# nianticlabs/simplerecon

Measured on AMD Instinct MI355X. Metric: depth frames/sec (640x480, 7 src views, 64 planes), higher is better.
Workload: dtype f32

## Files before the change

include/simplerecon_hip.h:

```cpp
#ifndef SIMPLERECON_HIP_H_
#define SIMPLERECON_HIP_H_

#include <stddef.h>
#include <stdint.h>

#ifdef __cplusplus
extern "C" {
#endif

#define SR_OK 0
#define SR_ERR_INVALID_ARGUMENT 1
#define SR_ERR_UNSUPPORTED 2
#define SR_ERR_WORKSPACE_TOO_SMALL 3
#define SR_ERR_HIP_BASE 1000

enum {
  SR_OPT_MLP_SPLIT = 0, SR_OPT_WINO_SPLIT, SR_OPT_WINO_XCD, SR_OPT_WINO_NT, SR_OPT_WINO_KSPLIT, SR_OPT_CONV_WINO,
  SR_OPT_CONV_TILE, SR_OPT_CONV_KSPLIT, SR_OPT_PW_NT, SR_OPT_PW_KS, SR_OPT_PT_CFG, SR_OPT_PT_KS, SR_OPT_DOT_LDS,
  SR_OPT_DOT_LDS_G, SR_OPT_DOT_LDS_CULL, SR_OPT_DOT_LDS_CAP, SR_OPT_UPSAMPLE_QUAD, SR_OPT_POOL_STREAM,
  SR_OPT_COUNT
};
int sr_option_count(void);
const char* sr_option_name(int id);
int sr_option_id(const char* name);
int sr_option_get(int id, int* value);
int sr_option_set(int id, int value, int* previous );
int sr_option_default(int id, int* value);

int sr_abi_version(void);

const char* sr_target_arch(void);


size_t sr_volume_workspace_bytes(int B, int K, int C, int h, int w);

int sr_volume_prepare(const float* src, const float* K_src, const float* T_src_cur,
                      const float* T_cur_src, int B, int K, int C, int h, int w, void* workspace,
                      size_t workspace_bytes, void* stream);

int sr_dot_volume_sweep(const float* cur, const float* invK_cur, const float* planes, int64_t ps_b,
                        int64_t ps_d, int64_t ps_y, int64_t ps_x, int B, int K, int C, int h, int w,
                        int D, float* out_cv, int64_t cv_sb, int64_t cv_sd, int64_t cv_sp,
                        float* out_lowest, uint8_t* out_mask, void* workspace,
                        size_t workspace_bytes, void* stream);

int sr_conv3x3_wino_io_nhwc_fwd(const void* in, int64_t in_batch_stride, int in_pix_stride, const float* packed_u,
                                const float* bias, const void* residual, int64_t res_batch_stride, int res_pix_stride,
                                void* out, int64_t out_batch_stride, int out_pix_stride, int B, int H, int W, int Cin,
                                int Cout, float leaky_slope, int io_dtype, void* stream);
int sr_pw_conv_io_nhwc_fwd(const void* in, int64_t in_batch_stride, int in_pix_stride, const float* packed_w,
                           const float* bias, const void* residual, int64_t res_batch_stride, int res_pix_stride, void* out,
                           int64_t out_batch_stride, int out_pix_stride, int B, int HW, int Cin, int Cout, float act_code,
                           int io_dtype, void* stream);

size_t sr_pw_conv_tiled_workspace_bytes(int M, int Cin, int Cout);
int sr_pw_conv_tiled_plan(int M, int Cin, int Cout, int can_split, int* cfg, int* ks);
int sr_pw_conv_tiled_nhwc_fwd(const float* in, int in_pix_stride, const float* packed_w, const float* bias,
                              const float* gate, const float* residual, int res_pix_stride, float* out,
                              int out_pix_stride, int M, int HW, int Cin, int Cout, float act_code, void* workspace,
                              size_t workspace_bytes, void* stream);
int sr_pw_conv_supported(int Cin, int Cout);
int sr_pw_conv_plan(int B, int HW, int Cin, int Cout, int* nt, int* ks);
int sr_pw_conv_nhwc_fwd(const float* in, int64_t in_batch_stride, int in_pix_stride, const float* packed_w,
                        const float* bias, const float* gate, const float* residual, int64_t res_batch_stride,
                        int res_pix_stride, float* out, int64_t out_batch_stride, int out_pix_stride, int B, int HW,
                        int Cin, int Cout, float act_code, void* stream);

int sr_backproject_fwd(const float* depth, const float* invK, float* out_points, int B, int h, int w, void* stream);
int sr_project3d_fwd(const float* points, const float* K, const float* T, float* out, int B, int N, float eps,
                     void* stream);
int sr_backproject_bwd(const float* grad_points, const float* invK, float* grad_depth, int B, int h, int w, void* stream);
int sr_project3d_bwd(const float* grad_out, const float* points, const float* K, const float* T, float* grad_points, int B,
// ... 416 lines not shown
```

simplerecon_amd/csrc/sr_options.hip:

```cpp
#include <atomic>
#include <mutex>
#include <stdlib.h>
#include <string.h>

#include "sr_common.h"

namespace {

struct OptDef { const char* name; int dflt; int kind; };
const OptDef kDefs[SR_OPT_COUNT] = {
    {"SR_MLP_SPLIT", 0, 1},       {"SR_WINO_SPLIT", 0, 1},     {"SR_WINO_XCD", 1, 0},        {"SR_WINO_NT", 0, 0},
    {"SR_WINO_KSPLIT", 0, 0},     {"SR_CONV_WINO", 1, 0},      {"SR_CONV_TILE", 0, 0},       {"SR_CONV_KSPLIT", 1, 0},
    {"SR_PW_NT", 0, 0},           {"SR_PW_KS", 0, 0},          {"SR_PT_CFG", -1, 0},         {"SR_PT_KS", 0, 0},
    {"SR_DOT_LDS", 1, 0},         {"SR_DOT_LDS_G", 0, 0},      {"SR_DOT_LDS_CULL", 1, 0},    {"SR_DOT_LDS_CAP", 634, 0},
    {"SR_UPSAMPLE_QUAD", 1, 0},   {"SR_POOL_STREAM", 1, 0},
};
std::atomic<int> g_val[SR_OPT_COUNT];
std::once_flag g_once;

int parse(const OptDef& d, const char* e) {
  if (d.kind == 1) {
    if (!e || !*e || !strcmp(e, "0") || !strcmp(e, "off") || !strcmp(e, "fp32")) return 0;
    if (!strcmp(e, "bf16")) return 1;
    if (!strcmp(e, "f16") || !strcmp(e, "fp16")) return 2;
    return -1;
  }
  return (e && *e) ? atoi(e) : d.dflt;
}

void init() {
  for (int i = 0; i < SR_OPT_COUNT; ++i) {
    const char* e = getenv(kDefs[i].name);
    g_val[i].store(e ? parse(kDefs[i], e) : kDefs[i].dflt, std::memory_order_relaxed);
  }
}

}

int sr_opt(int id) {
  std::call_once(g_once, init);
  return g_val[id].load(std::memory_order_relaxed);
}

extern "C" int sr_option_count(void) { return SR_OPT_COUNT; }

extern "C" const char* sr_option_name(int id) { return (id >= 0 && id < SR_OPT_COUNT) ? kDefs[id].name : nullptr; }

extern "C" int sr_option_id(const char* name) {
  if (!name) return -1;
  for (int i = 0; i < SR_OPT_COUNT; ++i)
    if (!strcmp(kDefs[i].name, name)) return i;
  return -1;
}

extern "C" int sr_option_get(int id, int* value) {
  if (id < 0 || id >= SR_OPT_COUNT || !value) return SR_ERR_INVALID_ARGUMENT;
  *value = sr_opt(id);
  return SR_OK;
}

extern "C" int sr_option_set(int id, int value, int* previous) {
  if (id < 0 || id >= SR_OPT_COUNT) return SR_ERR_INVALID_ARGUMENT;
  std::call_once(g_once, init);
  const int old = g_val[id].exchange(value, std::memory_order_relaxed);
  if (previous) *previous = old;
  return SR_OK;
}

// ... 19 lines not shown
```

simplerecon_amd/csrc/sr_pw.hip:

```cpp
#include <stdlib.h>

#include "sr_common.h"

namespace {

typedef float pw_f16 __attribute__((ext_vector_type(16)));
typedef float pw_f4 __attribute__((ext_vector_type(4)));
typedef unsigned int pw_u4 __attribute__((ext_vector_type(4)));
#define PW_RSRC_FLAGS 0x00020000
#define PW_OOB 0x7fffffffu

__device__ __forceinline__ pw_f4 pw_load(__amdgpu_buffer_rsrc_t r, unsigned voff, unsigned soff) {
  return __builtin_bit_cast(pw_f4, __builtin_amdgcn_raw_buffer_load_b128(r, (int)voff, (int)soff, 0));
}
typedef unsigned int pw_u2 __attribute__((ext_vector_type(2)));
template <int IO>
__device__ __forceinline__ float pw_widen(unsigned short h) {
  if (IO == 1) return (float)__builtin_bit_cast(_Float16, h);
  return __builtin_bit_cast(float, (unsigned)h << 16);
}
template <int IO>
__device__ __forceinline__ unsigned short pw_narrow(float f) {
  if (IO == 1) return __builtin_bit_cast(unsigned short, (_Float16)f);
  return __builtin_bit_cast(unsigned short, (__bf16)f);
}
template <int IO>
__device__ __forceinline__ pw_f4 pw_load_a(__amdgpu_buffer_rsrc_t r, unsigned voff, unsigned soff) {
  if (IO == 0) return __builtin_bit_cast(pw_f4, __builtin_amdgcn_raw_buffer_load_b128(r, (int)voff, (int)soff, 0));
  const pw_u2 v = __builtin_bit_cast(pw_u2, __builtin_amdgcn_raw_buffer_load_b64(r, (int)voff, (int)soff, 0));
  return pw_f4{pw_widen<IO>((unsigned short)(v.x & 0xffffu)), pw_widen<IO>((unsigned short)(v.x >> 16)),
               pw_widen<IO>((unsigned short)(v.y & 0xffffu)), pw_widen<IO>((unsigned short)(v.y >> 16))};
}
template <int IO>
__device__ __forceinline__ float pw_load_elem(__amdgpu_buffer_rsrc_t r, unsigned voff, unsigned soff) {
  if (IO == 0) return __builtin_bit_cast(float, __builtin_amdgcn_raw_buffer_load_b32(r, (int)voff, (int)soff, 0));
  return pw_widen<IO>(__builtin_amdgcn_raw_buffer_load_b16(r, (int)voff, (int)soff, 0));
}
template <int IO>
__device__ __forceinline__ void pw_store_elem(float v, __amdgpu_buffer_rsrc_t r, unsigned voff, unsigned soff) {
  if (IO == 0) __builtin_amdgcn_raw_buffer_store_b32(__builtin_bit_cast(unsigned, v), r, (int)voff, (int)soff, 0);
  else __builtin_amdgcn_raw_buffer_store_b16(pw_narrow<IO>(v), r, (int)voff, (int)soff, 0);
}
#define PW_ES(io) ((io) == 0 ? 4u : 2u)

__device__ __forceinline__ __amdgpu_buffer_rsrc_t pw_rsrc(const void* base, int64_t bytes) {
  return __builtin_amdgcn_make_buffer_rsrc(const_cast<void*>(base), 0, (int)bytes, PW_RSRC_FLAGS);
}

struct SrPwParams {
  const float* in; int64_t in_sb; int in_sp;
  const float* wp;
  const float* bias;
  const float* gate;
  const float* res; int64_t res_sb; int res_sp;
  float* out; int64_t out_sb; int out_sp;
  int B, HW, Cin, Cout, Co_pad, G, G8;
  int m_tiles, n_blocks, total_mt;
  float slope;
};

#ifndef SR_PW_U
#define SR_PW_U 4
#define SR_PW_PD 3
#endif
constexpr int PW_U = SR_PW_U;
constexpr int PW_PD = SR_PW_PD;

template <int NT, int KS, bool GATE, int IO = 0>
__global__ __launch_bounds__(256, 2) void sr_pw_kernel(SrPwParams p) {
  constexpr unsigned ES = PW_ES(IO);
  extern __shared__ __attribute__((aligned(16))) float red[];
  const int tid = threadIdx.x;
  const int lane = tid & 63, wave = __builtin_amdgcn_readfirstlane(tid >> 6);
  const int i = lane & 31, kk = lane >> 5;
  constexpr int MT_PER_WG = 4 / KS;
  const int ml = wave / KS, kp = wave % KS;
  const int item = blockIdx.x;
  const int nb = item % p.n_blocks;
  const int mt_g = (item / p.n_blocks) * MT_PER_WG + ml;
  const bool live = mt_g < p.total_mt;
  const int img = live ? mt_g / p.m_tiles : 0;
  const int row0 = live ? (mt_g - img * p.m_tiles) * 32 : 0;
  const int n0 = nb * (32 * NT);

  const int per = ((p.G8 + KS - 1) / KS + PW_U - 1) / PW_U * PW_U;
  const int g0 = kp * per;
  const int g1 = min(p.G8, g0 + per);
  const int steps = live && g1 > g0 ? (g1 - g0 + PW_U - 1) / PW_U * PW_U : 0;

  const __amdgpu_buffer_rsrc_t rs_in = pw_rsrc(reinterpret_cast<const char*>(p.in) + (int64_t)img * p.in_sb * ES,
                                               ((int64_t)(p.HW - 1) * p.in_sp + p.Cin) * ES);
  const __amdgpu_buffer_rsrc_t rs_w = pw_rsrc(p.wp, (int64_t)p.G * 2 * p.Co_pad * 16);
  const __amdgpu_buffer_rsrc_t rs_g = pw_rsrc(GATE ? p.gate + (int64_t)img * p.Cin : p.wp, GATE ? (int64_t)p.Cin * 4 : 0);
  const int row = row0 + i;
  const unsigned a_voff = (row < p.HW) ? ((unsigned)row * (unsigned)p.in_sp + 4u * kk) * ES : PW_OOB;
  const bool k_tail = (p.Cin & 7) != 0;
  const unsigned w_voff = (unsigned)(kk * p.Co_pad + n0 + i) * 16u;
  const unsigned g_voff = 16u * kk;
  const int g_last_w = p.G - 1;

  pw_f16 acc[NT];
#pragma unroll
  for (int n = 0; n < NT; ++n)
#pragma unroll
    for (int r = 0; r < 16; ++r) acc[n][r] = 0.0f;

  pw_f4 a_f[PW_U], b_f[PW_U][NT], s_f[PW_U];
  auto issue = [&](int g, int slot) {
    const bool in_range = g < g1;
    unsigned av = in_range ? a_voff : PW_OOB;
    if (k_tail && 8 * g + 4 * kk + 4 > p.Cin) av = PW_OOB;
    a_f[slot] = pw_load_a<IO>(rs_in, av, (unsigned)g * 8u * ES);
    if (GATE) s_f[slot] = pw_load(rs_g, g_voff + (unsigned)g * 32u, 0u);
    const unsigned gw = (unsigned)min(g, g_last_w);
#pragma unroll
    for (int n = 0; n < NT; ++n) b_f[slot][n] = pw_load(rs_w, w_voff + 512u * n, gw * 2u * (unsigned)p.Co_pad * 16u);
  };
  if (steps > 0) {
#pragma unroll
    for (int s = 0; s < PW_PD; ++s) issue(g0 + s, s);
  }
  for (int gb = 0; gb < steps; gb += PW_U) {
#pragma unroll
    for (int u = 0; u < PW_U; ++u) {
      issue(g0 + gb + u + PW_PD, (u + PW_PD) % PW_U);
      pw_f4 a = a_f[u];
      if (GATE) a = a * s_f[u];
#pragma unroll
      for (int e = 0; e < 4; ++e)
#pragma unroll
        for (int n = 0; n < NT; ++n) acc[n] = __builtin_amdgcn_mfma_f32_32x32x2f32(a[e], b_f[u][n][e], acc[n], 0, 0, 0);
    }
  }

  if (KS > 1) {
    if (kp > 0 && live) {
#pragma unroll
      for (int n = 0; n < NT; ++n)
// ... 170 lines not shown
```

simplerecon_amd/csrc/sr_pw_tiled.hip:

```cpp
#include <stdlib.h>

#include "sr_common.h"

namespace {

typedef float pt_f16 __attribute__((ext_vector_type(16)));
typedef float pt_f4 __attribute__((ext_vector_type(4)));

constexpr int PT_KS = 32;
constexpr int PT_AROW = PT_KS + 4;

struct SrPtParams {
  const float* in; int in_sp;
  const float* wp;
  const float* bias; const float* gate;
  const float* res; int res_sp;
  float* out; int out_sp;
  int64_t part_stride;
  int M, HW, Cin, Cout, Co_pad, G;
  int slabs, slabs_per_part, ksplit, tiles_n;
  float slope;
};

template <int WM, int WN, int NTW, bool GATE>
__global__ __launch_bounds__(256, 2) void sr_pw_tiled_kernel(SrPtParams p) {
  constexpr int BM = 32 * WM, BN = 32 * WN * NTW;
  constexpr int A_FLOATS = BM * PT_AROW, B_FLOATS = (PT_KS / 8) * 2 * BN * 4;
  constexpr int A_PER_THREAD = BM * (PT_KS / 4) / 256;
  constexpr int B_PER_THREAD = (PT_KS / 8) * 2 * BN / 256;
  static_assert(WM * WN == 4 && A_PER_THREAD >= 1 && B_PER_THREAD >= 1, "4 waves; whole float4s per thread");
  extern __shared__ __attribute__((aligned(16))) float lds[];
  const int tid = threadIdx.x, lane = tid & 63, wave = __builtin_amdgcn_readfirstlane(tid >> 6);
  const int i = lane & 31, kk = lane >> 5;
  const int wm = wave / WN, wn = wave % WN;
  const int tile_n = blockIdx.x % p.tiles_n, tile_m = blockIdx.x / p.tiles_n;
  const int kpart = blockIdx.y;
  const int m0 = tile_m * BM, n0 = tile_n * BN;
  const int s_begin = kpart * p.slabs_per_part, s_end = min(p.slabs, s_begin + p.slabs_per_part);

  int a_row[A_PER_THREAD];
  const float* a_ptr[A_PER_THREAD];
  const float* g_ptr[A_PER_THREAD];
  const int a_q = tid & 7;
#pragma unroll
  for (int u = 0; u < A_PER_THREAD; ++u) {
    a_row[u] = (tid >> 3) + 32 * u;
    const int m = m0 + a_row[u];
    const bool ok = m < p.M;
    a_ptr[u] = ok ? p.in + (int64_t)m * p.in_sp + 4 * a_q : nullptr;
    g_ptr[u] = (GATE && ok) ? p.gate + (int64_t)(m / p.HW) * p.Cin + 4 * a_q : nullptr;
  }
  auto stage_load = [&](int s, pt_f4 (&ra)[A_PER_THREAD], pt_f4 (&rb)[B_PER_THREAD]) {
    const int k0 = s * PT_KS;
#pragma unroll
    for (int u = 0; u < A_PER_THREAD; ++u) {
      pt_f4 v = {0.f, 0.f, 0.f, 0.f};
      if (a_ptr[u] && k0 + 4 * a_q < p.Cin) {
        v = *reinterpret_cast<const pt_f4*>(a_ptr[u] + k0);
        if (GATE) v = v * *reinterpret_cast<const pt_f4*>(g_ptr[u] + k0);
      }
      ra[u] = v;
    }
#pragma unroll
    for (int u = 0; u < B_PER_THREAD; ++u) {
      const int e = tid + 256 * u;
      const int gh = e / BN, col = e - gh * BN;
      const int g = s * (PT_KS / 8) + (gh >> 1);
      pt_f4 v = {0.f, 0.f, 0.f, 0.f};
      if (g < p.G && n0 + col < p.Co_pad)
        v = *reinterpret_cast<const pt_f4*>(p.wp + ((int64_t)(g * 2 + (gh & 1)) * p.Co_pad + n0 + col) * 4);
      rb[u] = v;
    }
  };
  auto stage_store = [&](int buf, const pt_f4 (&ra)[A_PER_THREAD], const pt_f4 (&rb)[B_PER_THREAD]) {
    float* A = lds + buf * (A_FLOATS + B_FLOATS);
    float* Bt = A + A_FLOATS;
#pragma unroll
    for (int u = 0; u < A_PER_THREAD; ++u) *reinterpret_cast<pt_f4*>(&A[a_row[u] * PT_AROW + 4 * a_q]) = ra[u];
#pragma unroll
    for (int u = 0; u < B_PER_THREAD; ++u) *reinterpret_cast<pt_f4*>(&Bt[(tid + 256 * u) * 4]) = rb[u];
  };

  pt_f16 acc[NTW];
#pragma unroll
  for (int n = 0; n < NTW; ++n)
#pragma unroll
    for (int r = 0; r < 16; ++r) acc[n][r] = 0.0f;

  pt_f4 ra[A_PER_THREAD], rb[B_PER_THREAD];
  if (s_begin < s_end) {
    stage_load(s_begin, ra, rb);
    stage_store(0, ra, rb);
  }
  __syncthreads();
  for (int s = s_begin; s < s_end; ++s) {
    const int buf = (s - s_begin) & 1;
    const bool more = s + 1 < s_end;
    if (more) stage_load(s + 1, ra, rb);
    const float* A = lds + buf * (A_FLOATS + B_FLOATS);
    const float* Bt = A + A_FLOATS;
    const float* a_base = A + (32 * wm + i) * PT_AROW + 4 * kk;
    const float* b_base = Bt + (kk * BN + 32 * wn * NTW + i) * 4;
#pragma unroll
    for (int gl = 0; gl < PT_KS / 8; ++gl) {
      const pt_f4 a = *reinterpret_cast<const pt_f4*>(a_base + 8 * gl);
      pt_f4 b[NTW];
#pragma unroll
      for (int n = 0; n < NTW; ++n) b[n] = *reinterpret_cast<const pt_f4*>(b_base + (gl * 2 * BN + 32 * n) * 4);
#pragma unroll
      for (int e = 0; e < 4; ++e)
#pragma unroll
        for (int n = 0; n < NTW; ++n) acc[n] = __builtin_amdgcn_mfma_f32_32x32x2f32(a[e], b[n][e], acc[n], 0, 0, 0);
    }
    if (more) stage_store(buf ^ 1, ra, rb);
    __syncthreads();
  }

  const bool partial = p.ksplit > 1;
  const float slope = sr_uniform(partial ? -1.0f : p.slope);
  float* outp = p.out + (partial ? (int64_t)kpart * p.part_stride : (int64_t)0);
  const int rbase = m0 + 32 * wm + 4 * kk;
#pragma unroll
  for (int n = 0; n < NTW; ++n) {
    const int col = n0 + 32 * (wn * NTW + n) + i;
    const bool okc = col < p.Cout;
    const float bv = (!partial && p.bias && okc) ? p.bias[col] : 0.0f;
    float v[16];
#pragma unroll
    for (int r = 0; r < 16; ++r) v[r] = acc[n][r] + bv;
    if (!partial && p.res) {
      float rv[16];
#pragma unroll
      for (int r = 0; r < 16; ++r) {
        const int m = rbase + (r & 3) + 8 * (r >> 2);
        rv[r] = (okc && m < p.M) ? p.res[(int64_t)m * p.res_sp + col] : 0.0f;
      }
#pragma unroll
      for (int r = 0; r < 16; ++r) v[r] += rv[r];
    }
    sr_activate_group(v, slope);
#pragma unroll
    for (int r = 0; r < 16; ++r) {
      const int m = rbase + (r & 3) + 8 * (r >> 2);
      if (okc && m < p.M) outp[(int64_t)m * p.out_sp + col] = v[r];
    }
  }
}

int pt_num_cus() { return sr_device_cus(); }

struct PtPlan { int cfg, ks; };
constexpr int PT_BM[4] = {64, 128, 128, 64}, PT_BN[4] = {128, 160, 64, 64};

PtPlan pt_plan(int M, int Cin, int Cout, bool can_split) {
  const int f_cfg = sr_opt(SR_OPT_PT_CFG), f_ks = sr_opt(SR_OPT_PT_KS);
  const int slabs = (Cin + PT_KS - 1) / PT_KS;
  const long want = (long)pt_num_cus() * 3 / 2;
  PtPlan best = {0, 1};
  double best_cost = -1.0;
  for (int cfg = 0; cfg < 4; ++cfg) {
    if (f_cfg >= 0 && cfg != f_cfg) continue;
    const long tm = (M + PT_BM[cfg] - 1) / PT_BM[cfg], tn = (Cout + PT_BN[cfg] - 1) / PT_BN[cfg];
    const double pad = (double)(tm * PT_BM[cfg]) * (double)(tn * PT_BN[cfg]) / ((double)M * Cout);
    for (int ks = 1; ks <= 8; ks *= 2) {
      if (f_ks > 0 && ks != f_ks) continue;
      if (ks > 1 && (!can_split || slabs / ks < 4)) continue;
      const long wgs = tm * tn * ks;
      const double fill = wgs >= want ? 1.0 : (double)want / (double)wgs;
      const double reuse = 1.0 + 24.0 / (PT_BM[cfg] * PT_BN[cfg] / (double)(PT_BM[cfg] + PT_BN[cfg]));
      const double cost = pad * fill * reuse * (1.0 + (ks > 1 ? 0.10 + 2.0 * ks / slabs : 0.0));
      if (best_cost < 0 || cost < best_cost) { best = {cfg, ks}; best_cost = cost; }
    }
  }
  return best;
}

template <int WM, int WN, int NTW>
int pt_launch(const SrPtParams& p, int tiles_m, hipStream_t stream) {
  constexpr int BM = 32 * WM, BN = 32 * WN * NTW;
  const size_t lds = (size_t)2 * (BM * PT_AROW + (PT_KS / 8) * 2 * BN * 4) * sizeof(float);
  const dim3 grid((unsigned)(tiles_m * p.tiles_n), (unsigned)p.ksplit);
  if (p.gate) {
    hipError_t e = hipFuncSetAttribute((const void*)sr_pw_tiled_kernel<WM, WN, NTW, true>,
                                       hipFuncAttributeMaxDynamicSharedMemorySize, (int)lds);
    if (e != hipSuccess) return sr_hip_rc(e);
    hipLaunchKernelGGL((sr_pw_tiled_kernel<WM, WN, NTW, true>), grid, dim3(256), lds, stream, p);
  } else {
    hipError_t e = hipFuncSetAttribute((const void*)sr_pw_tiled_kernel<WM, WN, NTW, false>,
                                       hipFuncAttributeMaxDynamicSharedMemorySize, (int)lds);
    if (e != hipSuccess) return sr_hip_rc(e);
    hipLaunchKernelGGL((sr_pw_tiled_kernel<WM, WN, NTW, false>), grid, dim3(256), lds, stream, p);
  }
  return sr_hip_rc(hipGetLastError());
}

}

extern "C" size_t sr_pw_conv_tiled_workspace_bytes(int M, int Cin, int Cout) {
  if (M <= 0 || Cin <= 0 || Cout <= 0 || Cout % 4 != 0) return 0;
  const PtPlan pl = pt_plan(M, Cin, Cout, true);
  return pl.ks > 1 ? (size_t)pl.ks * M * Cout * sizeof(float) : 0;
}

extern "C" int sr_pw_conv_tiled_plan(int M, int Cin, int Cout, int can_split, int* cfg, int* ks) {
  if (M <= 0 || Cin <= 0 || Cout <= 0) return SR_ERR_INVALID_ARGUMENT;
  const PtPlan pl = pt_plan(M, Cin, Cout, can_split != 0 && Cout % 4 == 0);
  if (cfg) *cfg = pl.cfg;
  if (ks) *ks = pl.ks;
  return SR_OK;
}

extern "C" int sr_pw_conv_tiled_nhwc_fwd(const float* in, int in_pix_stride, const float* packed_w, const float* bias,
                                         const float* gate, const float* residual, int res_pix_stride, float* out,
                                         int out_pix_stride, int M, int HW, int Cin, int Cout, float act_code,
                                         void* workspace, size_t workspace_bytes, void* stream_) {
  if (M < 0 || HW <= 0 || Cin <= 0 || Cout <= 0) return SR_ERR_INVALID_ARGUMENT;
  if (M == 0) return SR_OK;
  if (!in || !packed_w || !out) return SR_ERR_INVALID_ARGUMENT;
  if (Cin % 4 != 0 || in_pix_stride % 4 != 0 || (((uintptr_t)in) & 15) != 0 || (gate && (((uintptr_t)gate) & 15) != 0))
    return SR_ERR_UNSUPPORTED;
  const bool can_split = workspace && (((uintptr_t)workspace) & 15) == 0 && Cout % 4 == 0 &&
                         (!residual || ((((uintptr_t)residual) & 15) == 0 && res_pix_stride % 4 == 0)) &&
                         (((uintptr_t)out) & 15) == 0 && out_pix_stride % 4 == 0 && (!bias || (((uintptr_t)bias) & 15) == 0);
  PtPlan pl = pt_plan(M, Cin, Cout, can_split);
  if (pl.ks > 1 && workspace_bytes < (size_t)pl.ks * M * Cout * sizeof(float)) pl = pt_plan(M, Cin, Cout, false);
  SrPtParams p;
  p.in = in; p.in_sp = in_pix_stride; p.wp = packed_w; p.bias = bias; p.gate = gate;
  p.res = residual; p.res_sp = res_pix_stride;
  p.M = M; p.HW = HW; p.Cin = Cin; p.Cout = Cout;
  p.Co_pad = ((Cout + 31) / 32) * 32;
  p.G = ((Cin + 63) / 64) * 8;
  p.slabs = (Cin + PT_KS - 1) / PT_KS;
  p.ksplit = pl.ks;
  p.slabs_per_part = (p.slabs + pl.ks - 1) / pl.ks;
  p.slope = act_code;
  p.part_stride = (int64_t)M * Cout;
  if (pl.ks > 1) { p.out = (float*)workspace; p.out_sp = Cout; }
  else { p.out = out; p.out_sp = out_pix_stride; }
  const int tiles_m = (M + PT_BM[pl.cfg] - 1) / PT_BM[pl.cfg];
  p.tiles_n = (Cout + PT_BN[pl.cfg] - 1) / PT_BN[pl.cfg];
  hipStream_t stream = (hipStream_t)stream_;
  int rc;
  switch (pl.cfg) {
    case 0: rc = pt_launch<2, 2, 2>(p, tiles_m, stream); break;
    case 1: rc = pt_launch<4, 1, 5>(p, tiles_m, stream); break;
    case 2: rc = pt_launch<4, 1, 2>(p, tiles_m, stream); break;
    default: rc = pt_launch<2, 2, 1>(p, tiles_m, stream); break;
  }
  if (rc == SR_OK && pl.ks > 1)
    rc = sr_launch_splitk_reduce((const float*)workspace, pl.ks, p.part_stride, bias, residual, (int64_t)0, res_pix_stride,
                                 out, (int64_t)0, out_pix_stride, 1, M, Cout, act_code, stream);
  return rc;
}
```

simplerecon_amd/ops.py:

```python
import ctypes as C
import contextlib
import os
import weakref

import torch
from torch import nn

from . import _lib

PROFILE = None

_PACKED = weakref.WeakKeyDictionary()
_NO_ENTRIES = {}


def _cached(mod, tag, key, build, *args):
    e = _PACKED.get(mod, _NO_ENTRIES).get(tag)
    if e is not None and e[0] == key:
        if e[2] is not None:
            _await_pack(e)
        return e[1]
    payload = build(*args)
    fence = None
    if _lib.cuda_available() and not _lib.capturing():
# ... 91 lines not shown
        return (w._version, w.data_ptr(), b._version, b.data_ptr())
    ts = [w] if b is None else [w, b]
    bufs, bp = bn._buffers, bn._parameters
    ts += [bufs["running_mean"], bufs["running_var"]]
    if bn.affine:
        ts += [bp["weight"], bp["bias"]]
    return tuple((t._version, t.data_ptr()) if t is not None else None for t in ts)


def bn_affine(bn):
    if bn.running_mean is None or bn.running_var is None:
        raise _lib.HipLibraryError("BatchNorm without running statistics cannot run in inference mode")
    scale = torch.rsqrt(bn.running_var.detach() + bn.eps)
    if bn.affine:
        scale = scale * bn.weight.detach()
    shift = -bn.running_mean.detach() * scale
    if bn.affine:
        shift = shift + bn.bias.detach()
    return scale.contiguous(), shift.contiguous()


def _effective_weight(conv, bn):
    w = conv.weight.detach()
    b = conv.bias.detach() if conv.bias is not None else None
    if bn is not None:
        scale, shift = bn_affine(bn)
        w = w * scale.view(-1, 1, 1, 1)
        b = shift if b is None else b * scale + shift
    return w.contiguous(), b


def _check_conv(conv):
    k = conv.kernel_size[0]
    if conv.kernel_size[0] != conv.kernel_size[1] or k not in (1, 3) or conv.groups != 1 \
            or conv.dilation != (1, 1) or tuple(conv.padding) != (k // 2,) * 2 \
            or conv.padding_mode not in ("zeros", "replicate"):
        raise _lib.HipLibraryError(f"unsupported Conv2d configuration for the HIP path: {conv}")


def _pack_folded(kind, conv, bn):
    _lib.require_device_f32("conv weight", conv.weight)
    _check_conv(conv)
    w, bias = _effective_weight(conv, bn)
    return _pack(kind, w), bias


def packed_weight(conv: nn.Conv2d, bn=None):
    return _cached(conv, "direct", _state_key(conv, bn), _pack_folded, "conv", conv, bn)


USE_PW_1X1 = True
PW_TILED = os.environ.get("SR_PW_TILED", "auto")
PW_TILED_MIN_ROWS = 100000


def _pack_linear(lin):
    return _pack("conv", lin.weight.detach().reshape(lin.out_features, lin.in_features, 1, 1).contiguous())


def linear(x, lin: nn.Linear, leaky=None):
    _lib.require_device_f32("linear input", x)
    _lib.refuse_autograd(x, lin.weight)
    cin, cout = lin.in_features, lin.out_features
    if x.shape[-1] != cin:
        raise ValueError(f"linear expects {cin} input features, got {x.shape[-1]}")
    x2 = x.reshape(-1, cin).contiguous()
    m = x2.shape[0]
    out = torch.empty((m, cout), dtype=torch.float32, device=x.device)
    if m == 0:
        return out.view(*x.shape[:-1], cout)
    wp = _cached(lin, "linear", _state_key(lin, None), _pack_linear, lin)
    bias = lin.bias.detach() if lin.bias is not None else None
    _lib.call("sr_conv2d_nhwc_fwd", x.device, x2, m * cin, cin, wp, bias, None, 0, 0, out, m * cout, cout, 1, 1, m, cin, cout,
              1, 1, -1.0 if leaky is None else float(leaky))
    return out.view(*x.shape[:-1], cout)


def wino_split_mode():
    return _lib.split_mode_name("SR_WINO_SPLIT")


def packed_wino_weight(conv: nn.Conv2d, bn=None):
    key = (_state_key(conv, bn), wino_split_mode())
    return _cached(conv, "wino", key, _pack_folded, "wino", conv, bn)


WINO4_MODE = int(os.environ.get("SR_CONV_WINO4", "1"))
WINO4_VARIANT = int(os.environ.get("SR_WINO4_VARIANT", "0"))


def packed_wino4_weight(conv: nn.Conv2d, bn=None):
    return _cached(conv, "wino4", _state_key(conv, bn), _pack_folded, "wino4", conv, bn)


_SHAPE_QUERIES = {}


def _drop_shape_queries(*_):
    _SHAPE_QUERIES.clear()


_lib.OPTION_LISTENERS.append(_drop_shape_queries)


def _shape_query(lib, name, *shape, dev=None):
    key = (name, shape, dev)
# ... 72 lines not shown
            if _conv_wino(lib, x, *packed_wino_weight(conv, bn), residual, out, strides, shape, slope) == 0:
                return out
        finally:
            _lib.SPLIT_GUARD.release()
        wp, bias = packed_weight(conv, bn)
        isb, isp, osb, osp, rsb, rsp = strides
        _lib.call("sr_conv2d_nhwc_fwd", x.device, x, isb, isp, wp, bias, residual, rsb, rsp, out, osb, osp, b, h, w, ci, co,
                  k, s, slope)
        return out
    _conv_direct(lib, x, *packed_weight(conv, bn), residual, out, strides, shape, slope, pads if padded else None, replicate)
    return out


def _aligned16(t, sb, sp):
    return t is None or (t.data_ptr() % 16 == 0 and sp % 4 == 0 and sb % 4 == 0)


def _timed(device, record, fn, *args):
    prof = PROFILE
    with _lib.on_device(device):
        if prof is None:
            return fn(*args)
        ev0, ev1 = torch.cuda.Event(enable_timing=True), torch.cuda.Event(enable_timing=True)
        ev0.record()
        rc = fn(*args)
        ev1.record()
        if rc == 0:
            name, flops, shape, executed = record()
            prof.append((name, flops, ev0, ev1, shape, executed))
    return rc


def _launch(x, shape, entry, fallback, describe, fn, *args):
    if PROFILE is None:
        with _lib.on_device(x.device):
            rc = fn(*args)
    else:
        def record():
            b, ci, h, w, co, k, s, ho, wo, _ = shape
            name, executed = describe()
            return name, 2.0 * b * ho * wo * co * ci * k * k, shape, executed
        rc = _timed(x.device, record, fn, *args)
    if rc != 0 and (rc != _lib.ERR_UNSUPPORTED or not fallback):
        _lib.check(rc, entry)
    return rc


def _conv_pointwise(lib, x, wp, bias, residual, out, gate, strides, shape, slope):
    isb, isp, osb, osp, rsb, rsp = strides
    b, ci, h, w, co = shape[:5]
    m = b * h * w
    dense = b == 1 or (isb == h * w * isp and osb == h * w * osp and (residual is None or rsb == h * w * rsp))
    gflag = "true" if gate is not None else "false"
    if dense and (PW_TILED == "1" or (PW_TILED == "auto" and m >= PW_TILED_MIN_ROWS)):
        nbytes = _shape_query(lib, "sr_pw_conv_tiled_workspace_bytes", m, ci, co, dev=x.device.index)
        ws = _workspace(x.device, "pw_splitk", nbytes) if nbytes else None

        def describe():
            a_, b_ = C.c_int(0), C.c_int(0)
            can_split = ws is not None and ws.data_ptr() % 16 == 0 and co % 4 == 0 and _aligned16(out, 0, osp) and \
                _aligned16(residual, 0, rsp) and (bias is None or bias.data_ptr() % 16 == 0)
            lib.sr_pw_conv_tiled_plan(m, ci, co, int(can_split), C.byref(a_), C.byref(b_))
            if b_.value > 1 and nbytes < b_.value * m * co * 4:
                lib.sr_pw_conv_tiled_plan(m, ci, co, 0, C.byref(a_), C.byref(b_))
            tile_m, tile_n = ((64, 128), (128, 160), (128, 64), (64, 64))[a_.value]
            executed = 2.0 * (-(-m // tile_m) * tile_m) * (-(-co // tile_n) * tile_n) * (-(-ci // 32) * 32)
            return f"sr_pw_tiled_kernel<{tile_m}x{tile_n}, ks {b_.value}, {gflag}>", executed
        return _launch(x, shape, "sr_pw_conv_tiled_nhwc_fwd", gate is None, describe, lib.sr_pw_conv_tiled_nhwc_fwd,
                       _lib.ptr(x), isp, _lib.ptr(wp), _lib.ptr(bias), _lib.ptr(gate), _lib.ptr(residual), rsp, _lib.ptr(out),
                       osp, m, h * w, ci, co, slope, _lib.ptr(ws), nbytes, _lib.stream_ptr(x.device))

    def describe():
        a_, b_ = C.c_int(0), C.c_int(0)
        lib.sr_pw_conv_plan(b, h * w, ci, co, C.byref(a_), C.byref(b_))
        mt = b * ((h * w + 31) // 32)
        executed = 2.0 * mt * 32 * ((co + 32 * a_.value - 1) // (32 * a_.value) * 32 * a_.value) * ((ci + 7) // 8 * 8)
        return f"sr_pw_kernel<{a_.value}, {b_.value}, {gflag}>", executed
    return _launch(x, shape, "sr_pw_conv_nhwc_fwd", gate is None, describe, lib.sr_pw_conv_nhwc_fwd, _lib.ptr(x), isb, isp,
                   _lib.ptr(wp), _lib.ptr(bias), _lib.ptr(gate), _lib.ptr(residual), rsb, rsp, _lib.ptr(out), osb, osp, b,
                   h * w, ci, co, slope, _lib.stream_ptr(x.device))


def _conv_wino4(lib, x, wp, bias, residual, out, strides, shape, slope, variant):
    isb, isp, osb, osp, rsb, rsp = strides
    b, ci, h, w, co = shape[:5]
    if not (_aligned16(x, isb, isp) and _aligned16(out, osb, osp) and _aligned16(residual, rsb, rsp)
            and (bias is None or bias.data_ptr() % 16 == 0)):
        return _lib.ERR_UNSUPPORTED

    def describe():
        regions = ((h + 15) // 16) * ((w + 15) // 16)
        executed = 2.0 * b * regions * 16 * 36 * ((ci + 15) // 16 * 16) * ((co + 63) // 64 * 64)
        return "sr_wino4ws_kernel" if variant == 3 else "sr_wino4_kernel", executed
    return _launch(x, shape, "sr_conv3x3_wino4_nhwc_fwd", True, describe, lib.sr_conv3x3_wino4_variant_nhwc_fwd, _lib.ptr(x),
                   isb, isp, _lib.ptr(wp), _lib.ptr(bias), _lib.ptr(residual), rsb, rsp, _lib.ptr(out), osb, osp, b, h, w, ci,
                   co, slope, variant, _lib.stream_ptr(x.device))


def _conv_wino(lib, x, wp, bias, residual, out, strides, shape, slope, workspace=True, fallback=True):
    isb, isp, osb, osp, rsb, rsp = strides
    b, ci, h, w, co = shape[:5]
    split = wino_split_mode()
    nbytes = _shape_query(lib, "sr_wino_splitk_workspace_bytes", b, h, w, ci, co, dev=x.device.index) if workspace else 0
    ws = _workspace(x.device, "wino_splitk", nbytes) if nbytes else None

    def describe():
        vin = bool(_aligned16(x, isb, isp) and ci % 4 == 0)
# ... 401 lines not shown
```

Measured before the change: 313.6.

## Rework tiled pointwise conv pipeline, planner cost model, and gated routing

Adds a configurable register-set prefetch depth to the tiled pointwise kernel. Loads become unconditional with clamped addresses and masking moves to the LDS store. The tile/split-k planner gets a new analytic cost model that tries every ks from 1 to 8, and hipFuncSetAttribute is cached per device. Gated 1x1 convs with large Cin and mid-size M are now routed to the tiled kernel, and the simple pw kernel's K-partition alignment is decoupled from its unroll factor. Default depth stays 1, so the main default-path changes are the restructured load/store masking, the new planner and the new routing.

```diff
diff --git a/include/simplerecon_hip.h b/include/simplerecon_hip.h
--- a/include/simplerecon_hip.h
+++ b/include/simplerecon_hip.h
@@ -18,6 +18,7 @@
   SR_OPT_MLP_SPLIT = 0, SR_OPT_WINO_SPLIT, SR_OPT_WINO_XCD, SR_OPT_WINO_NT, SR_OPT_WINO_KSPLIT, SR_OPT_CONV_WINO,
   SR_OPT_CONV_TILE, SR_OPT_CONV_KSPLIT, SR_OPT_PW_NT, SR_OPT_PW_KS, SR_OPT_PT_CFG, SR_OPT_PT_KS, SR_OPT_DOT_LDS,
   SR_OPT_DOT_LDS_G, SR_OPT_DOT_LDS_CULL, SR_OPT_DOT_LDS_CAP, SR_OPT_UPSAMPLE_QUAD, SR_OPT_POOL_STREAM,
+  SR_OPT_PT_DEPTH,
   SR_OPT_COUNT
 };
 int sr_option_count(void);
diff --git a/simplerecon_amd/csrc/sr_options.hip b/simplerecon_amd/csrc/sr_options.hip
--- a/simplerecon_amd/csrc/sr_options.hip
+++ b/simplerecon_amd/csrc/sr_options.hip
@@ -13,7 +13,7 @@
     {"SR_WINO_KSPLIT", 0, 0},     {"SR_CONV_WINO", 1, 0},      {"SR_CONV_TILE", 0, 0},       {"SR_CONV_KSPLIT", 1, 0},
     {"SR_PW_NT", 0, 0},           {"SR_PW_KS", 0, 0},          {"SR_PT_CFG", -1, 0},         {"SR_PT_KS", 0, 0},
     {"SR_DOT_LDS", 1, 0},         {"SR_DOT_LDS_G", 0, 0},      {"SR_DOT_LDS_CULL", 1, 0},    {"SR_DOT_LDS_CAP", 634, 0},
-    {"SR_UPSAMPLE_QUAD", 1, 0},   {"SR_POOL_STREAM", 1, 0},
+    {"SR_UPSAMPLE_QUAD", 1, 0},   {"SR_POOL_STREAM", 1, 0},    {"SR_PT_DEPTH", 0, 0},
 };
 std::atomic<int> g_val[SR_OPT_COUNT];
 std::once_flag g_once;
diff --git a/simplerecon_amd/csrc/sr_pw.hip b/simplerecon_amd/csrc/sr_pw.hip
--- a/simplerecon_amd/csrc/sr_pw.hip
+++ b/simplerecon_amd/csrc/sr_pw.hip
@@ -59,15 +59,19 @@
   float slope;
 };
 
-#ifndef SR_PW_U
-#define SR_PW_U 4
-#define SR_PW_PD 3
+template <int NT> struct PwPipe { static constexpr int U = 4, PD = 3; };
+#ifdef SR_PW_U
+#define PW_PIPE_U(NT) SR_PW_U
+#define PW_PIPE_PD(NT) SR_PW_PD
+#else
+#define PW_PIPE_U(NT) PwPipe<NT>::U
+#define PW_PIPE_PD(NT) PwPipe<NT>::PD
 #endif
-constexpr int PW_U = SR_PW_U;
-constexpr int PW_PD = SR_PW_PD;
-
-template <int NT, int KS, bool GATE, int IO = 0>
+constexpr int PW_KALIGN = 4;
+
+template <int NT, int KS, bool GATE, int IO = 0, int PW_U = PW_PIPE_U(NT), int PW_PD = PW_PIPE_PD(NT)>
 __global__ __launch_bounds__(256, 2) void sr_pw_kernel(SrPwParams p) {
+  static_assert(PW_PD >= 1 && PW_PD < PW_U, "loads run ahead within the rotating sets");
   constexpr unsigned ES = PW_ES(IO);
   extern __shared__ __attribute__((aligned(16))) float red[];
   const int tid = threadIdx.x;
@@ -83,7 +87,7 @@
   const int row0 = live ? (mt_g - img * p.m_tiles) * 32 : 0;
   const int n0 = nb * (32 * NT);
 
-  const int per = ((p.G8 + KS - 1) / KS + PW_U - 1) / PW_U * PW_U;
+  const int per = ((p.G8 + KS - 1) / KS + PW_KALIGN - 1) / PW_KALIGN * PW_KALIGN;
   const int g0 = kp * per;
   const int g1 = min(p.G8, g0 + per);
   const int steps = live && g1 > g0 ? (g1 - g0 + PW_U - 1) / PW_U * PW_U : 0;
diff --git a/simplerecon_amd/csrc/sr_pw_tiled.hip b/simplerecon_amd/csrc/sr_pw_tiled.hip
--- a/simplerecon_amd/csrc/sr_pw_tiled.hip
+++ b/simplerecon_amd/csrc/sr_pw_tiled.hip
@@ -1,3 +1,4 @@
+#include <atomic>
 #include <stdlib.h>
 
 #include "sr_common.h"
@@ -22,13 +23,15 @@
   float slope;
 };
 
-template <int WM, int WN, int NTW, bool GATE>
+template <int WM, int WN, int NTW, bool GATE, int D>
 __global__ __launch_bounds__(256, 2) void sr_pw_tiled_kernel(SrPtParams p) {
   constexpr int BM = 32 * WM, BN = 32 * WN * NTW;
   constexpr int A_FLOATS = BM * PT_AROW, B_FLOATS = (PT_KS / 8) * 2 * BN * 4;
   constexpr int A_PER_THREAD = BM * (PT_KS / 4) / 256;
   constexpr int B_PER_THREAD = (PT_KS / 8) * 2 * BN / 256;
+  constexpr int G_PER_THREAD = GATE ? A_PER_THREAD : 1;
   static_assert(WM * WN == 4 && A_PER_THREAD >= 1 && B_PER_THREAD >= 1, "4 waves; whole float4s per thread");
+  static_assert(D >= 1 && D <= 3, "register sets");
   extern __shared__ __attribute__((aligned(16))) float lds[];
   const int tid = threadIdx.x, lane = tid & 63, wave = __builtin_amdgcn_readfirstlane(tid >> 6);
   const int i = lane & 31, kk = lane >> 5;
@@ -37,48 +40,58 @@
   const int kpart = blockIdx.y;
   const int m0 = tile_m * BM, n0 = tile_n * BN;
   const int s_begin = kpart * p.slabs_per_part, s_end = min(p.slabs, s_begin + p.slabs_per_part);
+  const int nslab = max(s_end - s_begin, 0);
 
   int a_row[A_PER_THREAD];
+  bool a_ok[A_PER_THREAD];
   const float* a_ptr[A_PER_THREAD];
-  const float* g_ptr[A_PER_THREAD];
+  const float* g_ptr[G_PER_THREAD];
   const int a_q = tid & 7;
 #pragma unroll
   for (int u = 0; u < A_PER_THREAD; ++u) {
     a_row[u] = (tid >> 3) + 32 * u;
     const int m = m0 + a_row[u];
-    const bool ok = m < p.M;
-    a_ptr[u] = ok ? p.in + (int64_t)m * p.in_sp + 4 * a_q : nullptr;
-    g_ptr[u] = (GATE && ok) ? p.gate + (int64_t)(m / p.HW) * p.Cin + 4 * a_q : nullptr;
-  }
-  auto stage_load = [&](int s, pt_f4 (&ra)[A_PER_THREAD], pt_f4 (&rb)[B_PER_THREAD]) {
-    const int k0 = s * PT_KS;
+    a_ok[u] = m < p.M;
+    const int mc = min(m, p.M - 1);
+    a_ptr[u] = p.in + (int64_t)mc * p.in_sp;
+    if (GATE) g_ptr[u] = p.gate + (int64_t)(mc / p.HW) * p.Cin;
+  }
+  int b_off[B_PER_THREAD];
+#pragma unroll
+  for (int u = 0; u < B_PER_THREAD; ++u) {
+    const int e = tid + 256 * u;
+    const int gh = e / BN, col = e - gh * BN;
+    b_off[u] = n0 + col < p.Co_pad ? (gh * p.Co_pad + n0 + col) * 4 : -1;
+  }
+  const int b_slab = (PT_KS / 8) * 2 * p.Co_pad * 4;
+  auto stage_load = [&](int s, pt_f4 (&ra)[A_PER_THREAD], pt_f4 (&rg)[G_PER_THREAD], pt_f4 (&rb)[B_PER_THREAD]) {
+    s = min(s, p.slabs - 1);
+    const int k = s * PT_KS + 4 * a_q;
+    const int kc = k < p.Cin ? k : 0;
 #pragma unroll
     for (int u = 0; u < A_PER_THREAD; ++u) {
-      pt_f4 v = {0.f, 0.f, 0.f, 0.f};
-      if (a_ptr[u] && k0 + 4 * a_q < p.Cin) {
-        v = *reinterpret_cast<const pt_f4*>(a_ptr[u] + k0);
-        if (GATE) v = v * *reinterpret_cast<const pt_f4*>(g_ptr[u] + k0);
-      }
-      ra[u] = v;
+      ra[u] = *reinterpret_cast<const pt_f4*>(a_ptr[u] + kc);
+      if (GATE) rg[u] = *reinterpret_cast<const pt_f4*>(g_ptr[u] + kc);
     }
 #pragma unroll
     for (int u = 0; u < B_PER_THREAD; ++u) {
-      const int e = tid + 256 * u;
-      const int gh = e / BN, col = e - gh * BN;
-      const int g = s * (PT_KS / 8) + (gh >> 1);
-      pt_f4 v = {0.f, 0.f, 0.f, 0.f};
-      if (g < p.G && n0 + col < p.Co_pad)
-        v = *reinterpret_cast<const pt_f4*>(p.wp + ((int64_t)(g * 2 + (gh & 1)) * p.Co_pad + n0 + col) * 4);
-      rb[u] = v;
+      rb[u] = *reinterpret_cast<const pt_f4*>(p.wp + (int64_t)s * b_slab + max(b_off[u], 0));
     }
   };
-  auto stage_store = [&](int buf, const pt_f4 (&ra)[A_PER_THREAD], const pt_f4 (&rb)[B_PER_THREAD]) {
+  auto stage_store = [&](int s, int buf, const pt_f4 (&ra)[A_PER_THREAD], const pt_f4 (&rg)[G_PER_THREAD],
+                         const pt_f4 (&rb)[B_PER_THREAD]) {
     float* A = lds + buf * (A_FLOATS + B_FLOATS);
     float* Bt = A + A_FLOATS;
-#pragma unroll
-    for (int u = 0; u < A_PER_THREAD; ++u) *reinterpret_cast<pt_f4*>(&A[a_row[u] * PT_AROW + 4 * a_q]) = ra[u];
-#pragma unroll
-    for (int u = 0; u < B_PER_THREAD; ++u) *reinterpret_cast<pt_f4*>(&Bt[(tid + 256 * u) * 4]) = rb[u];
+    const pt_f4 zero = {0.f, 0.f, 0.f, 0.f};
+    const bool k_ok = s * PT_KS + 4 * a_q < p.Cin;
+#pragma unroll
+    for (int u = 0; u < A_PER_THREAD; ++u) {
+      pt_f4 v = ra[u];
+      if (GATE) v = v * rg[u];
+      *reinterpret_cast<pt_f4*>(&A[a_row[u] * PT_AROW + 4 * a_q]) = (a_ok[u] && k_ok) ? v : zero;
+    }
+#pragma unroll
+    for (int u = 0; u < B_PER_THREAD; ++u) *reinterpret_cast<pt_f4*>(&Bt[(tid + 256 * u) * 4]) = b_off[u] >= 0 ? rb[u] : zero;
   };
 
   pt_f16 acc[NTW];
@@ -87,35 +100,40 @@
 #pragma unroll
     for (int r = 0; r < 16; ++r) acc[n][r] = 0.0f;
 
-  pt_f4 ra[A_PER_THREAD], rb[B_PER_THREAD];
-  if (s_begin < s_end) {
-    stage_load(s_begin, ra, rb);
-    stage_store(0, ra, rb);
-  }
+  pt_f4 ra[D][A_PER_THREAD], rg[D][G_PER_THREAD], rb[D][B_PER_THREAD];
+#pragma unroll
+  for (int d = 0; d < D; ++d)
+    if (D > 1 || d < nslab) stage_load(s_begin + d, ra[d], rg[d], rb[d]);
+  if (nslab > 0) stage_store(s_begin, 0, ra[0], rg[0], rb[0]);
   __syncthreads();
-  for (int s = s_begin; s < s_end; ++s) {
-    const int buf = (s - s_begin) & 1;
-    const bool more = s + 1 < s_end;
-    if (more) stage_load(s + 1, ra, rb);
-    const float* A = lds + buf * (A_FLOATS + B_FLOATS);
-    const float* Bt = A + A_FLOATS;
-    const float* a_base = A + (32 * wm + i) * PT_AROW + 4 * kk;
-    const float* b_base = Bt + (kk * BN + 32 * wn * NTW + i) * 4;
-#pragma unroll
-    for (int gl = 0; gl < PT_KS / 8; ++gl) {
-      const pt_f4 a = *reinterpret_cast<const pt_f4*>(a_base + 8 * gl);
-      pt_f4 b[NTW];
-#pragma unroll
-      for (int n = 0; n < NTW; ++n) b[n] = *reinterpret_cast<const pt_f4*>(b_base + (gl * 2 * BN + 32 * n) * 4);
-#pragma unroll
-      for (int e = 0; e < 4; ++e)
-#pragma unroll
-        for (int n = 0; n < NTW; ++n) acc[n] = __builtin_amdgcn_mfma_f32_32x32x2f32(a[e], b[n][e], acc[n], 0, 0, 0);
-    }
-    if (more) stage_store(buf ^ 1, ra, rb);
-    __syncthreads();
-  }
-
+  for (int j0 = 0; j0 < nslab; j0 += D) {
+#pragma unroll
+    for (int u = 0; u < D; ++u) {
+      const int j = j0 + u;
+      if (D > 1 || j + D < nslab) stage_load(s_begin + j + D, ra[u], rg[u], rb[u]);
+      __builtin_amdgcn_sched_barrier(0);
+      if (j < nslab) {
+        const float* A = lds + (j & 1) * (A_FLOATS + B_FLOATS);
+        const float* Bt = A + A_FLOATS;
+        const float* a_base = A + (32 * wm + i) * PT_AROW + 4 * kk;
+        const float* b_base = Bt + (kk * BN + 32 * wn * NTW + i) * 4;
+#pragma unroll
+        for (int gl = 0; gl < PT_KS / 8; ++gl) {
+          const pt_f4 a = *reinterpret_cast<const pt_f4*>(a_base + 8 * gl);
+          pt_f4 b[NTW];
+#pragma unroll
+          for (int n = 0; n < NTW; ++n) b[n] = *reinterpret_cast<const pt_f4*>(b_base + (gl * 2 * BN + 32 * n) * 4);
+#pragma unroll
+          for (int e = 0; e < 4; ++e)
+#pragma unroll
+            for (int n = 0; n < NTW; ++n) acc[n] = __builtin_amdgcn_mfma_f32_32x32x2f32(a[e], b[n][e], acc[n], 0, 0, 0);
+        }
+        __builtin_amdgcn_sched_barrier(0);
+        if (j + 1 < nslab) stage_store(s_begin + j + 1, (j + 1) & 1, ra[(u + 1) % D], rg[(u + 1) % D], rb[(u + 1) % D]);
+        __syncthreads();
+      }
+    }
+  }
   const bool partial = p.ksplit > 1;
   const float slope = sr_uniform(partial ? -1.0f : p.slope);
   float* outp = p.out + (partial ? (int64_t)kpart * p.part_stride : (int64_t)0);
@@ -152,46 +170,73 @@
 struct PtPlan { int cfg, ks; };
 constexpr int PT_BM[4] = {64, 128, 128, 64}, PT_BN[4] = {128, 160, 64, 64};
 
+constexpr int PT_DEPTH[2][4] = {{1, 1, 1, 1}, {1, 1, 1, 1}};
+int pt_depth(int cfg, bool gated) {
+  const int f = sr_opt(SR_OPT_PT_DEPTH);
+  return f > 0 ? (f < 3 ? f : 3) : PT_DEPTH[gated ? 1 : 0][cfg];
+}
+
+constexpr double PT_T_SLAB = 0.64;
+constexpr double PT_T_LOAD = 0.00056;
+constexpr double PT_T_SPLIT = 1.5;
+constexpr double PT_T_PART = 1.6e-6;
+
 PtPlan pt_plan(int M, int Cin, int Cout, bool can_split) {
   const int f_cfg = sr_opt(SR_OPT_PT_CFG), f_ks = sr_opt(SR_OPT_PT_KS);
   const int slabs = (Cin + PT_KS - 1) / PT_KS;
-  const long want = (long)pt_num_cus() * 3 / 2;
+  const long cus = pt_num_cus();
   PtPlan best = {0, 1};
   double best_cost = -1.0;
   for (int cfg = 0; cfg < 4; ++cfg) {
     if (f_cfg >= 0 && cfg != f_cfg) continue;
     const long tm = (M + PT_BM[cfg] - 1) / PT_BM[cfg], tn = (Cout + PT_BN[cfg] - 1) / PT_BN[cfg];
-    const double pad = (double)(tm * PT_BM[cfg]) * (double)(tn * PT_BN[cfg]) / ((double)M * Cout);
-    for (int ks = 1; ks <= 8; ks *= 2) {
+    for (int ks = 1; ks <= 8; ++ks) {
       if (f_ks > 0 && ks != f_ks) continue;
       if (ks > 1 && (!can_split || slabs / ks < 4)) continue;
+      const int per_part = (slabs + ks - 1) / ks;
+      if (f_ks <= 0 && (ks - 1) * per_part >= slabs) continue;
       const long wgs = tm * tn * ks;
-      const double fill = wgs >= want ? 1.0 : (double)want / (double)wgs;
-      const double reuse = 1.0 + 24.0 / (PT_BM[cfg] * PT_BN[cfg] / (double)(PT_BM[cfg] + PT_BN[cfg]));
-      const double cost = pad * fill * reuse * (1.0 + (ks > 1 ? 0.10 + 2.0 * ks / slabs : 0.0));
+      const long rounds = (wgs + cus - 1) / cus;
+      double cost = PT_T_SLAB * (double)rounds * (PT_BM[cfg] * PT_BN[cfg] / 4096.0) * per_part +
+                    PT_T_LOAD * (double)wgs * per_part * ((PT_BM[cfg] + PT_BN[cfg]) / 128.0);
+      if (ks > 1) cost += PT_T_SPLIT + PT_T_PART * ks * (double)M * Cout;
       if (best_cost < 0 || cost < best_cost) { best = {cfg, ks}; best_cost = cost; }
     }
   }
   return best;
 }
 
-template <int WM, int WN, int NTW>
-int pt_launch(const SrPtParams& p, int tiles_m, hipStream_t stream) {
+template <int WM, int WN, int NTW, bool GATE, int D>
+int pt_launch_depth(const SrPtParams& p, int tiles_m, hipStream_t stream) {
   constexpr int BM = 32 * WM, BN = 32 * WN * NTW;
-  const size_t lds = (size_t)2 * (BM * PT_AROW + (PT_KS / 8) * 2 * BN * 4) * sizeof(float);
-  const dim3 grid((unsigned)(tiles_m * p.tiles_n), (unsigned)p.ksplit);
-  if (p.gate) {
-    hipError_t e = hipFuncSetAttribute((const void*)sr_pw_tiled_kernel<WM, WN, NTW, true>,
+  constexpr size_t lds = (size_t)2 * (BM * PT_AROW + (PT_KS / 8) * 2 * BN * 4) * sizeof(float);
+  constexpr int kMaxDevices = 64;
+  static std::atomic<bool> prepared[kMaxDevices];
+  int dev = 0;
+  const bool cached = hipGetDevice(&dev) == hipSuccess && dev >= 0 && dev < kMaxDevices;
+  if (!cached || !prepared[dev].load(std::memory_order_acquire)) {
+    hipError_t e = hipFuncSetAttribute((const void*)sr_pw_tiled_kernel<WM, WN, NTW, GATE, D>,
                                        hipFuncAttributeMaxDynamicSharedMemorySize, (int)lds);
     if (e != hipSuccess) return sr_hip_rc(e);
-    hipLaunchKernelGGL((sr_pw_tiled_kernel<WM, WN, NTW, true>), grid, dim3(256), lds, stream, p);
-  } else {
-    hipError_t e = hipFuncSetAttribute((const void*)sr_pw_tiled_kernel<WM, WN, NTW, false>,
-                                       hipFuncAttributeMaxDynamicSharedMemorySize, (int)lds);
-    if (e != hipSuccess) return sr_hip_rc(e);
-    hipLaunchKernelGGL((sr_pw_tiled_kernel<WM, WN, NTW, false>), grid, dim3(256), lds, stream, p);
-  }
+    if (cached) prepared[dev].store(true, std::memory_order_release);
+  }
+  const dim3 grid((unsigned)(tiles_m * p.tiles_n), (unsigned)p.ksplit);
+  hipLaunchKernelGGL((sr_pw_tiled_kernel<WM, WN, NTW, GATE, D>), grid, dim3(256), lds, stream, p);
   return sr_hip_rc(hipGetLastError());
+}
+
+template <int WM, int WN, int NTW, bool GATE>
+int pt_launch_gate(const SrPtParams& p, int tiles_m, int depth, hipStream_t stream) {
+  constexpr int max_depth = NTW == 5 ? 2 : 3;
+  if (depth <= 1) return pt_launch_depth<WM, WN, NTW, GATE, 1>(p, tiles_m, stream);
+  if (depth == 2 || max_depth == 2) return pt_launch_depth<WM, WN, NTW, GATE, 2>(p, tiles_m, stream);
+  return pt_launch_depth<WM, WN, NTW, GATE, max_depth>(p, tiles_m, stream);
+}
+
+template <int WM, int WN, int NTW>
+int pt_launch(const SrPtParams& p, int tiles_m, int depth, hipStream_t stream) {
+  return p.gate ? pt_launch_gate<WM, WN, NTW, true>(p, tiles_m, depth, stream)
+                : pt_launch_gate<WM, WN, NTW, false>(p, tiles_m, depth, stream);
 }
 
 }
@@ -240,12 +285,13 @@
   const int tiles_m = (M + PT_BM[pl.cfg] - 1) / PT_BM[pl.cfg];
   p.tiles_n = (Cout + PT_BN[pl.cfg] - 1) / PT_BN[pl.cfg];
   hipStream_t stream = (hipStream_t)stream_;
+  const int depth = pt_depth(pl.cfg, gate != nullptr);
   int rc;
   switch (pl.cfg) {
-    case 0: rc = pt_launch<2, 2, 2>(p, tiles_m, stream); break;
-    case 1: rc = pt_launch<4, 1, 5>(p, tiles_m, stream); break;
-    case 2: rc = pt_launch<4, 1, 2>(p, tiles_m, stream); break;
-    default: rc = pt_launch<2, 2, 1>(p, tiles_m, stream); break;
+    case 0: rc = pt_launch<2, 2, 2>(p, tiles_m, depth, stream); break;
+    case 1: rc = pt_launch<4, 1, 5>(p, tiles_m, depth, stream); break;
+    case 2: rc = pt_launch<4, 1, 2>(p, tiles_m, depth, stream); break;
+    default: rc = pt_launch<2, 2, 1>(p, tiles_m, depth, stream); break;
   }
   if (rc == SR_OK && pl.ks > 1)
     rc = sr_launch_splitk_reduce((const float*)workspace, pl.ks, p.part_stride, bias, residual, (int64_t)0, res_pix_stride,
diff --git a/simplerecon_amd/ops.py b/simplerecon_amd/ops.py
--- a/simplerecon_amd/ops.py
+++ b/simplerecon_amd/ops.py
@@ -167,6 +167,10 @@
 USE_PW_1X1 = True
 PW_TILED = os.environ.get("SR_PW_TILED", "auto")
 PW_TILED_MIN_ROWS = 100000
+
+
+def _pw_prefers_tiled(m, ci, co, gated):
+    return gated and ci >= 960 and co % 4 == 0 and 2048 <= m <= 16384
 
 
 def _pack_linear(lin):
@@ -345,7 +349,8 @@
     m = b * h * w
     dense = b == 1 or (isb == h * w * isp and osb == h * w * osp and (residual is None or rsb == h * w * rsp))
     gflag = "true" if gate is not None else "false"
-    if dense and (PW_TILED == "1" or (PW_TILED == "auto" and m >= PW_TILED_MIN_ROWS)):
+    if dense and (PW_TILED == "1" or (PW_TILED == "auto" and (m >= PW_TILED_MIN_ROWS or
+                                                              _pw_prefers_tiled(m, ci, co, gate is not None)))):
         nbytes = _shape_query(lib, "sr_pw_conv_tiled_workspace_bytes", m, ci, co, dev=x.device.index)
         ws = _workspace(x.device, "pw_splitk", nbytes) if nbytes else None
 
```

New measurement: 313.9, median of 6. No clear change (+0.1%).
